# anguswilliams91/bpl-next

Hardware: NVIDIA B200
Metric: logdensity_grad_match_evals_per_s (higher is better)
Workload: dtype f32

## Files before the change

bpl_next_b200/csrc/api.cu:

```cuda
#include <limits.h>
#include <stdarg.h>
#include <stdlib.h>
#include <string.h>

#include <algorithm>
#include <atomic>
#include <mutex>
#include <new>

#include "common.cuh"
#include "plan.h"
#include "problem.h"
#include "loo.h"
#include "score_grid.h"
#include "simulate.h"

namespace bplx {

static thread_local char g_err[1024] = "";
static std::atomic<unsigned long long> g_launches{0};

void set_error(const char* fmt, ...) {
  va_list ap;
  va_start(ap, fmt);
// ... 216 lines not shown
  }
  p->kp = hp.kp;
  p->layout = hp.layout;
  p->lik_off = hp.lik_off;
  for (int i = 0; i < 12; i++) p->lik_hyper[i] = hp.lik_hyper[i];
  p->lik_nhyper = hp.lik_nhyper;
  p->lik_D = hp.lik_D;
  p->lik_const = hp.lik_const;
  p->lik_layout = hp.lik_layout;
  KernelParams& kp = p->kp;
#define UP(vec, ptr)                                 \
  if ((rc = upload(p, hp.vec, &(ptr))) != BPLX_OK) return fail(rc)
  UP(stream1, p->s1[0]);
  UP(stream2, p->s2[0]);
  UP(warp_b1, p->wb1[0]);
  UP(warp_b2, p->wb2[0]);
  for (int i = 1; i < kNumSplits; i++) {
    if (hp.more[i - 1].stream1.empty()) continue;
    UP(more[i - 1].stream1, p->s1[i]);
    UP(more[i - 1].stream2, p->s2[i]);
    UP(more[i - 1].warp_b1, p->wb1[i]);
    UP(more[i - 1].warp_b2, p->wb2[i]);
  }
  auto keep_bounds = [&](int i, const std::vector<uint32_t>& b1, const std::vector<uint32_t>& b2) {
    const size_t cap = sizeof(p->wb[i].b1) / sizeof(uint32_t);
    for (size_t k = 0; k < b1.size() && k < cap; k++) p->wb[i].b1[k] = b1[k];
    for (size_t k = 0; k < b2.size() && k < cap; k++) p->wb[i].b2[k] = b2[k];
  };
  keep_bounds(0, hp.warp_b1, hp.warp_b2);
  for (int i = 1; i < kNumSplits; i++) keep_bounds(i, hp.more[i - 1].warp_b1, hp.more[i - 1].warp_b2);
  kp.stream1 = p->s1[0];
  kp.stream2 = p->s2[0];
  kp.warp_b1 = p->wb1[0];
  kp.warp_b2 = p->wb2[0];
  kp.split = 1;
  UP(team_vptr, kp.team_vptr);
  UP(team_flags, kp.team_flags);
  UP(v_team, kp.v_team);
  UP(v_conf, kp.v_conf);
  UP(conf_vptr, kp.conf_vptr);
  UP(conf_vlist, kp.conf_vlist);
  UP(yexp, kp.yexp);
  UP(yteam, kp.yteam);
  UP(yconf, kp.yconf);
  UP(Xs, kp.Xs);
  UP(gw_tptr, kp.gw_tptr);
  UP(gw_tlist, kp.gw_tlist);
#undef UP
  rc = kp.model == BPLX_DYNAMIC ? logdensity_dynamic_set_attributes() : logdensity_set_attributes(kp);
  if (rc != BPLX_OK) return fail(rc);
  if (cudaDeviceGetAttribute(&p->sm_count, cudaDevAttrMultiProcessorCount, p->device) != cudaSuccess) p->sm_count = 0;
  p->max_clusters[0] = 1 << 30;
  if (kp.model != BPLX_DYNAMIC)
// ... 804 lines not shown
```

bpl_next_b200/csrc/k1_common.cuh:

```cuda
#pragma once
#include <float.h>

#include "common.cuh"
#include "plan.h"

namespace bplx {

namespace {


constexpr float kLn2 = 0.693147180559945309f;
constexpr unsigned kFull = 0xffffffffu;

struct Hyp {
  float mu_d, sig_a, sig_d, mu[4], sig[4];
};

struct Lane {
  const float* th;
  float* gr;
  float* sc;
  int sd;
  bool active;
  __device__ __forceinline__ float ld(int d) const { return __ldg(th + (uint32_t)(d * sd)); }
// ... 82 lines not shown
  const ThetaOffsets& o = kp.off;
  const float ra = g[eAh1] + g[eAa1] + g[eA0];
  const float rd = -(g[eBh1] + g[eBa1] + g[eB0]);
  const float rx[4] = {g[eAh1], g[eAa1], -g[eBh1], -g[eBa1]};
  if (kp.ndec == 0) hacc += rx[0];
  if (!ln.active) return;
  if (ADD) {
    red_add(ln.g(o.za + t), ra);
    red_add(ln.g(o.zd + t), rd);
  } else {
    *ln.g(o.za + t) = ra;
    *ln.g(o.zd + t) = rd;
  }
#pragma unroll
  for (int i = 0; i < 4; i++) {
    if (i < kp.ndec) {
      if (ADD) red_add(ln.g(o.dec[i] + t), rx[i]);
      else *ln.g(o.dec[i] + t) = rx[i];
    }
  }
}

__device__ __forceinline__ void put_side(const KernelParams& kp, float* q, const float (&g)[6], float& hacc) {
  q[0] = g[eAh1] + g[eAa1] + g[eA0];
  q[32] = -(g[eBh1] + g[eBa1] + g[eB0]);
  const float rx[4] = {g[eAh1], g[eAa1], -g[eBh1], -g[eBa1]};
  if (kp.ndec == 0) hacc += rx[0];
#pragma unroll
  for (int i = 0; i < 4; i++)
    if (i < kp.ndec) q[(2 + i) * 32] = rx[i];
}

struct Ring {
  uint32_t ring, bar;
  uint32_t S;
  const unsigned char* src;
  uint32_t total;
  uint32_t gs0, gs_next;
  int lane;

  __device__ __forceinline__ void init(uint32_t ring_, uint32_t bar_, uint32_t S_, int lane_) {
    ring = ring_; bar = bar_; S = S_; lane = lane_;
    total = gs0 = gs_next = 0;
    src = nullptr;
    if (lane == 0) {
#pragma unroll
      for (int s = 0; s < kStages; s++) mbar_init(bar + 8 * s, 1);
      fence_mbar_init();
      fence_proxy_async();
    }
    __syncwarp();
  }
  __device__ __forceinline__ void issue(uint32_t k) {
// ... 150 lines not shown
```

bpl_next_b200/csrc/logdensity.cu:

```cuda
#include <cooperative_groups.h>

#include <math.h>

#include "k1_common.cuh"
#include "problem.h"

namespace cg = cooperative_groups;

#ifdef BPLX_TIMELINE
__device__ unsigned long long g_timeline[32 * 24];
#define BPLX_STAMP(i)                                                                    \
  do {                                                                                   \
    if (blockIdx.x == 0 && (threadIdx.x & 31) == 0) {                                    \
      unsigned long long t_;                                                             \
      asm volatile("mov.u64 %0, %%globaltimer;" : "=l"(t_));                             \
      g_timeline[(threadIdx.x >> 5) * 24 + (i)] = t_;                                    \
    }                                                                                    \
  } while (0)
#define BPLX_STAMP_DEP(i, dep)                                                           \
  do {                                                                                   \
    if (blockIdx.x == 0 && (threadIdx.x & 31) == 0) {                                    \
      unsigned long long t_;                                                             \
      asm volatile("mov.u64 %0, %%globaltimer;" : "=l"(t_) : "f"(dep));                  \
      g_timeline[(threadIdx.x >> 5) * 24 + (i)] = t_;                                    \
    }                                                                                    \
// ... 60 lines not shown
    else __syncthreads();
  };
  const int chain_raw = group * kChains + lane;
  const int chain = min(chain_raw, kp.C - 1);
  Lane ln;
  ln.th = kp.theta + (size_t)chain * (size_t)kp.sc;
  ln.gr = kp.grad + (size_t)chain * (size_t)kp.sc;
  ln.sc = kp.scratch + chain;
  ln.sd = kp.sd;
  ln.active = chain_raw < kp.C;
  const uint32_t tab = smem_u32(smem) + lane * 8;
  unsigned long long* red_best = reinterpret_cast<unsigned long long*>(smem + kp.smem_red);
  unsigned long long* red_found = reinterpret_cast<unsigned long long*>(smem + kp.smem_red + 768);
  float* red_hyp = reinterpret_cast<float*>(smem + kp.smem_red + 1280);
  float* red_gc = reinterpret_cast<float*>(smem + kp.smem_red + 1280 + 12 * 128);
  const uint32_t a_best = cluster_map(smem_u32(red_best), 0), a_found = cluster_map(smem_u32(red_found), 0);
  const uint32_t a_cl = cluster_map(smem_u32(smem) + kp.smem_red_cl, 0);
  const uint32_t a_partcl = cluster_map(smem_u32(smem) + kp.epi_cl, 0);
  const uint32_t a_teamrows = cluster_map(smem_u32(smem) + kp.epi_team, 0);
  constexpr uint32_t ESZ = CLIP ? (uint32_t)sizeof(EntryClip) : (uint32_t)sizeof(Entry);
  Ring ring;
  ring.init(smem_u32(smem) + kp.smem_ring + warp * (kStages * kp.stage_bytes),
            smem_u32(smem) + kp.smem_bar + warp * (kStages * 8), kp.stage_bytes, lane);
  const uint32_t b1_0 = wb.b1[vwarp], b1_1 = wb.b1[vwarp + 1];
  ring.begin(kp.stream1 + b1_0, b1_1 - b1_0);
  pdl_wait();
  pdl_launch_dependents();
  ln.th = after_wait(ln.th);
  ln.gr = after_wait(ln.gr);
  ln.sc = after_wait(ln.sc);
  const int ndec = kp.ndec;
  const bool dc = ndec == 0;
  const float raw_in = ln.ld(o.raw);
  const bool lik = kp.lik_only != 0;
  const float u_in = (warp == 0 && !dc && !lik) ? ln.ld(o.u) : 0.0f;
  struct TeamIn { float za, zd, dz[4], xs[4]; int fl, v0, v1; };
  auto load_team = [&](int t) {
    TeamIn in;
    in.za = ln.ld(o.za + t);
    in.zd = ln.ld(o.zd + t);
#pragma unroll
    for (int i = 0; i < 4; i++) in.dz[i] = i < ndec ? ln.ld(o.dec[i] + t) : 0.0f;
#pragma unroll
    for (int j = 0; j < 4; j++) in.xs[j] = j < kp.K ? __ldg(kp.Xs + (size_t)t * kp.K + j) : 0.0f;
    in.fl = __ldg(kp.team_flags + t);
    in.v0 = __ldg(kp.team_vptr + t);
    in.v1 = __ldg(kp.team_vptr + t + 1);
    return in;
// ... 69 lines not shown
      for (int j = 0; j < 4; j++) {
        am = fmaf(in.xs[j], ba[j], am);
        dm = fmaf(in.xs[j], bd[j], dm);
      }
      for (int k = 4; k < kp.K; k++) {
        const float x = __ldg(kp.Xs + (size_t)t * kp.K + k);
        am = fmaf(x, ln.ld(o.beta_a + k), am);
        dm = fmaf(x, ln.ld(o.beta_d + k), dm);
      }
      const float att = fmaf(in.za, hy.sig_a, am), def = fmaf(in.zd, hy.sig_d, dm);
      float x[4] = {dc ? hy.mu[0] : 0.0f, 0.0f, 0.0f, 0.0f};
#pragma unroll
      for (int i = 0; i < 4; i++)
        if (i < ndec) x[i] = fmaf(hy.sig[i], in.dz[i], hy.mu[i]);
      if (!(in.fl & 1) && ln.active && crank == 0) {
        *ln.g(o.za + t) = 0.0f;
        *ln.g(o.zd + t) = 0.0f;
#pragma unroll
        for (int i = 0; i < 4; i++)
          if (i < ndec) *ln.g(o.dec[i] + t) = 0.0f;
      }
      for (int v = in.v0; v < in.v1; v++) {
        const float cf = kp.Cf > 0 ? ln.ld(o.conf + __ldg(kp.v_conf + v)) : 0.0f;
        float ex[6];
        ex[eAh1] = att + x[0] + cf;
        ex[eBh1] = -def - x[2] - cf;
        ex[eBa1] = -def - x[3] - cf;
        ex[eAa1] = att + x[1] + cf;
        ex[eA0] = att + cf;
        ex[eB0] = -def - cf;
        const uint32_t r = (uint32_t)v * kRowBytes;
        if (kp.has1) {
          sts64(tab + kp.tabP1 + r, expf(ex[eAh1]), expf(ex[eBh1]));
          sts64(tab + kp.tabQ1 + r, expf(ex[eBa1]), expf(ex[eAa1]));
        }
        if (kp.has0) sts64(tab + kp.tabP0 + r, expf(ex[eA0]), expf(ex[eB0]));
        if (CLIP) {
          exA = fmaxf(exA, fmaxf(ex[eAh1], fmaxf(ex[eAa1], ex[eA0])));
          exB = fmaxf(exB, fmaxf(ex[eBh1], fmaxf(ex[eBa1], ex[eB0])));
        }
        if (!CLIP && crank == 0) {
#pragma unroll
          for (int e = 0; e < 6; e++) lp_acc = fmaf(__ldg(kp.yexp + (size_t)v * 6 + e), ex[e], lp_acc);
        }
      }
    }
// ... 11 lines not shown
  bool fast1 = false;
  if (CLIP) fast1 = __all_sync(kFull, key_float(red_clip[lane]) + key_float(red_clip[32 + lane]) < 2.707f) && !(kp.force_clip_forms & 1);
  float best[3] = {0.0f, 0.0f, 0.0f};
  uint32_t besth[3] = {0u, 0u, 0u};
  {
    float g[6] = {0.0f, 0.0f, 0.0f, 0.0f, 0.0f, 0.0f}, cacc = 0.0f;
    const uint32_t nst = ring.num_stages();
    for (uint32_t k = 0; k < nst; k++) {
      uint32_t bytes;
      const uint32_t a0 = ring.acquire(k, &bytes);
      if (k == 0) BPLX_STAMP(16);
      uint32_t a = a0;
      const uint32_t aend = a0 + bytes;
      while (a + kp.min_piece1 <= aend) {
        const uint32_t hoff = b1_0 + k * ring.S + (a - a0);
        const Hdr L = unpack_hdr(lds128u(a));
        a += 16;
        const uint32_t e_end = a + L.n0 * ESZ;
        if (L.flags & kTeamFirst) {
#pragma unroll
          for (int e = 0; e < 6; e++) g[e] = 0.0f;
        }
        float2 own = lds64(tab + L.own_off);
        if (L.kind >= kH0) { const float s = own.x; own.x = own.y; own.y = s; }
        const bool home = (L.kind & 1) == 0;
        float gx, gy;
        if (!CLIP) {
          float2 acc0 = make_float2(0.0f, 0.0f), acc1 = acc0;
          if (home) {
            float m1 = 0.0f, m2 = 0.0f, m3 = 0.0f;
            walk16(a, e_end, [&](const uint32_t at) {
              const uint4 q = lds128u(at);
              const float2 ea = lds64(tab + q.x), eb = lds64(tab + q.z);
              acc0 = fma2(bc2(__uint_as_float(q.y)), ea, acc0);
              acc1 = fma2(bc2(__uint_as_float(q.w)), eb, acc1);
              m1 = fmaxf(m1, fmaxf(ea.x, eb.x));
              m2 = fmaxf(m2, fmaxf(ea.y, eb.y));
              m3 = fmaxf(m3, fmaxf(ea.x * ea.y, eb.x * eb.y));
            });
            const float v0 = own.x * m1, v1 = own.y * m2, v2 = (own.x * own.y) * m3;
            if (v0 > best[0]) { best[0] = v0; besth[0] = hoff; }
            if (v1 > best[1]) { best[1] = v1; besth[1] = hoff; }
            if (v2 > best[2]) { best[2] = v2; besth[2] = hoff; }
          } else {
            walk16(a, e_end, [&](const uint32_t at) {
              const uint4 q = lds128u(at);
              const float2 ea = lds64(tab + q.x), eb = lds64(tab + q.z);
              acc0 = fma2(bc2(__uint_as_float(q.y)), ea, acc0);
              acc1 = fma2(bc2(__uint_as_float(q.w)), eb, acc1);
            });
          }
          const float SX = own.x * (acc0.x + acc1.x), SY = own.y * (acc0.y + acc1.y);
          lp_acc -= 0.5f * (SX + SY);
          gx = -SX;
          gy = -SY;
        } else {
          float lp = 0.0f, m1 = 0.0f, m2 = 0.0f, m3 = 0.0f;
          if (fast1) {
            if (home) rate_piece_clip<true, true>(a, e_end, own, tab, lp, m1, m2, m3, gx, gy);
            else rate_piece_clip<true, false>(a, e_end, own, tab, lp, m1, m2, m3, gx, gy);
          } else {
            if (home) rate_piece_clip<false, true>(a, e_end, own, tab, lp, m1, m2, m3, gx, gy);
            else rate_piece_clip<false, false>(a, e_end, own, tab, lp, m1, m2, m3, gx, gy);
          }
          if (home) {
            lp_acc += lp;
            if (m1 > best[0]) { best[0] = m1; besth[0] = hoff; }
            if (m2 > best[1]) { best[1] = m2; besth[1] = hoff; }
            if (m3 > best[2]) { best[2] = m3; besth[2] = hoff; }
          }
        }
        add_own(g, L.kind, gx, gy);
        if (kp.Cf > 0) {
          cacc += L.kind == kH1 ? gx - gy : gy - gx;
          if (L.flags & kVteamLast) {
            if (ln.active) ln.sc[(size_t)L.vteam * kp.Cpad] = cacc;
            cacc = 0.0f;
          }
        }
        if (L.flags & kTeamLast) put_raw<false>(kp, ln, (int)L.team, g, hacc);
        if (k == 0 && a - a0 <= kp.stage_bytes / 2) BPLX_STAMP(17);
      }
      ring.release(k);
    }
  }
  const uint32_t b2_0 = wb.b2[vwarp], b2_1 = wb.b2[vwarp + 1];
  ring.begin(kp.stream2 + b2_0, b2_1 - b2_0);

  BPLX_STAMP(3);
#pragma unroll
  for (int q = 0; q < 3; q++)
    if (best[q] > 0.0f) dsm_atom_max_u32(a_best + (uint32_t)(q * 32 + lane) * 4u, __float_as_uint(best[q]));
  sync_all();
  BPLX_STAMP(14);
#pragma unroll
  for (int q = 0; q < 3; q++) {
    const float gq = __uint_as_float(dsm_ld_u32(a_best + (uint32_t)(q * 32 + lane) * 4u));
    if (best[q] == gq && gq > 0.0f) dsm_atom_min_u32(a_best + (uint32_t)((3 + q) * 32 + lane) * 4u, besth[q]);
    best[q] = gq;
  }
  sync_all();
  BPLX_STAMP(15);
#pragma unroll
  for (int q = 0; q < 3; q++) besth[q] = dsm_ld_u32(a_best + (uint32_t)((3 + q) * 32 + lane) * 4u);
  const bool noclip = CLIP && __all_sync(kFull, best[0] < 15.0f && best[1] < 15.0f) && !(kp.force_clip_forms & 2);
  const float Lam = fmaxf(best[0], best[1]);
  const int qlam = best[0] >= best[1] ? 0 : 1;
  bool s_need[2];
  uint32_t s_hoff[2], s_off0[2];
  uint4 s_hdr[2];
// ... 33 lines not shown
        float val;
        if (CLIP) {
          const float Xc = fminf(X, 15.0f), Yc = fminf(Y, 15.0f);
          val = q == 0 ? Xc : (q == 1 ? Yc : Xc * Yc);
        } else {
          val = q == 0 ? X : (q == 1 ? Y : (own.x * own.y) * (ea.x * ea.y));
        }
        if (val == target && found == 0xffffffffu) {
          found = (i << 24) | ((!CLIP || X < 15.0f) ? 1u << 23 : 0u) | ((!CLIP || Y < 15.0f) ? 1u << 22 : 0u) | off;
          info = L.vteam | (L.kind << 16);
        }
      }
    }
    if (found != 0xffffffffu) {
      dsm_atom_min_u32(a_found + (uint32_t)(which * 32 + lane) * 4u, found);
      dsm_st_u32(a_found + (uint32_t)(64 + which * 32 + lane) * 4u, info);
    }
  }

  BPLX_STAMP(5);
  float gc = 0.0f;
  {
    float g[6] = {0.0f, 0.0f, 0.0f, 0.0f, 0.0f, 0.0f}, cacc = 0.0f;
    const uint32_t nst = ring.num_stages();
    for (uint32_t k = 0; k < nst; k++) {
      uint32_t bytes;
      const uint32_t a0 = ring.acquire(k, &bytes);
      if (k == 0) BPLX_STAMP(18);
      uint32_t a = a0;
      const uint32_t aend = a0 + bytes;
      while (a + kp.min_piece2 <= aend) {
        const Hdr L = unpack_hdr(lds128u(a));
        a += 16;
        if (L.flags & kTeamFirst) {
#pragma unroll
          for (int e = 0; e < 6; e++) g[e] = 0.0f;
        }
        float2 own = lds64(tab + L.own_off);
        if (L.kind >= kH0) { const float s = own.x; own.x = own.y; own.y = s; }
        const bool home = (L.kind & 1) == 0;
        float lt, du, gx, gy;
        if (!CLIP) tau_piece<kTauPlain>(a, L, own, home, cc, tab, lt, du, gx, gy);
        else if (noclip) tau_piece<kTauUnclipped>(a, L, own, home, cc, tab, lt, du, gx, gy);
        else tau_piece<kTauClipped>(a, L, own, home, cc, tab, lt, du, gx, gy);
        if (home) {
          lp_acc = fmaf(lt, kLn2, lp_acc);
          gc += du;
        }
        add_own(g, L.kind, gx, gy);
        if (kp.Cf > 0) {
          cacc += L.kind == kH1 ? gx - gy : gy - gx;
          if (L.flags & kVteamLast) {
            if (ln.active) red_add(ln.sc + (size_t)L.vteam * kp.Cpad, cacc);
            cacc = 0.0f;
          }
        }
        if (L.flags & kTeamLast) {
          if (p2s) put_side(kp, p2_tab + (((L.kind & 1) * kp.T + L.team) * (2 + ndec)) * 32 + lane, g, hacc);
          else put_raw<true>(kp, ln, (int)L.team, g, hacc);
        }
      }
      ring.release(k);
    }
  }
  BPLX_STAMP(6);
  red_gc[warp * 32 + lane] = gc;
  __syncthreads();
  gc = 0.0f;
  for (int w = 0; w < W; w++) gc += red_gc[w * 32 + lane];
  if (S > 1) {
    if (warp == 0) dsm_st_f32(a_cl + (uint32_t)(crank * 32 + lane) * 4u, gc);
    cg::this_cluster().sync();
    gc = 0.0f;
    for (int q = 0; q < S; q++) gc += dsm_ld_f32(a_cl + (uint32_t)(q * 32 + lane) * 4u);
  }
  {
    const float t11 = fmaxf(1.0f - cc, 0.0f);
    gc -= kp.w11 / t11;
    if (vwarp == 0 && kp.w11 != 0.0f) lp_acc = fmaf(kp.w11, logf(t11), lp_acc);
  }

  BPLX_STAMP(7);
  Fixup fx;
  fx.h1 = 0u;
  fx.confs = 0u;
#pragma unroll
// ... 283 lines not shown
```

bpl_next_b200/csrc/plan.cc:

```cpp
#include "plan.h"

#include <algorithm>
#include <cmath>
#include <cstdarg>
#include <cstdio>
#include <cstdlib>
#include <cstring>
#include <map>
#include <numeric>

namespace bplx {
namespace {

struct RawEntry {
  uint32_t opp;
  uint8_t cls;
  double w, wyx, wyy;
};

std::string fmt(const char* f, ...) {
  char buf[512];
  va_list ap;
  va_start(ap, f);
  vsnprintf(buf, sizeof buf, f, ap);
// ... 309 lines not shown
  };
  auto opp_base = [&](int kind) -> uint32_t { return kind == kH1 ? kp.tabQ1 : kind == kA1 ? kp.tabP1 : kp.tabP0; };

  auto merge = [](std::vector<RawEntry>& v) {
    std::stable_sort(v.begin(), v.end(), [](const RawEntry& a, const RawEntry& b) {
      return a.cls != b.cls ? a.cls < b.cls : a.opp < b.opp;
    });
    size_t o = 0;
    for (size_t i = 0; i < v.size(); i++) {
      if (o && v[o - 1].cls == v[i].cls && v[o - 1].opp == v[i].opp) {
        v[o - 1].w += v[i].w;
        v[o - 1].wyx += v[i].wyx;
        v[o - 1].wyy += v[i].wyy;
      } else {
        v[o++] = v[i];
      }
    }
    v.resize(o);
  };
  for (auto& v : raw1) merge(v);
  for (auto& v : raw2) merge(v);
  P.team_flags.assign(T, 0);
  for (int v = 0; v < V; v++)
    for (int k = 0; k < 4; k++)
      if (!raw1[(size_t)v * 4 + k].empty()) P.team_flags[P.v_team[v]] |= 1;

  auto team_costs = [&](const std::vector<std::vector<RawEntry>>& raw, double per_entry, double per_list,
                        double per_team) {
    std::vector<double> cost(T, 0.0);
    for (int v = 0; v < V; v++)
      for (int k = 0; k < 4; k++) {
        const size_t n = raw[(size_t)v * 4 + k].size();
        if (n) cost[P.v_team[v]] += per_list * (1.0 + (double)n / 100.0) + per_entry * (double)n;
      }
    for (int t = 0; t < T; t++)
      if (cost[t] > 0.0) cost[t] += per_team;
    return cost;
  };
  auto assign = [&](const std::vector<double>& cost, int W, std::vector<std::vector<int>>* teams) {
    std::vector<int> order(T);
    std::iota(order.begin(), order.end(), 0);
    std::stable_sort(order.begin(), order.end(), [&](int a, int b) { return cost[a] > cost[b]; });
    std::vector<double> load(W, 0.0);
    teams->assign(W, {});
    for (int t : order) {
      if (cost[t] == 0.0) continue;
      int best = 0;
      for (int w = 1; w < W; w++)
        if (load[w] < load[best]) best = w;
      load[best] += cost[t];
      (*teams)[best].push_back(t);
    }
    for (auto& v : *teams) std::sort(v.begin(), v.end());
    return *std::max_element(load.begin(), load.end());
  };
  const std::vector<double> cost1 = team_costs(raw1, kp.clip ? 16.0 : 6.0, 40.0, 30.0);
  const std::vector<double> cost2 = team_costs(raw2, 12.0, 60.0, 30.0);
  auto smem_need = [&](int W, uint32_t stage) {
    const uint32_t epi = (K > 0 ? (uint32_t)T * kRowBytes : 0u) + (uint32_t)(W + kMaxSplit) * kPartRows * 128u;
    const uint32_t tabb = (std::max(table_bytes, epi) + 127u) / 128u * 128u;
    return tabb + (uint32_t)W * kStages * stage + 128u + (uint32_t)W * kStages * 8u + 3u * 256u + 2u * 128u + 2u * 128u +
           12u * 128u + (uint32_t)(W + kMaxSplit) * 128u;
  };
  const uint32_t kSmemMax = 227u * 1024u;
  int W = 0;
  uint32_t stage = 1024;
  std::vector<std::vector<int>> w1, w2;
  if (force_warps <= 0) {
    if (const char* e = getenv("BPLX_NWARPS")) force_warps = atoi(e);
  }
  if (const char* e = getenv("BPLX_STAGE")) stage = (uint32_t)atoi(e) == 512u ? 512u : 1024u;
  if (force_warps > 0) {
    W = std::max(1, std::min(force_warps, kMaxWarps));
    if (smem_need(W, stage) > kSmemMax) stage = 512;
  } else {
    double best = 0.0;
    for (int cand : {4, 8, 12, 16, 20, 24}) {
      if (cand > kMaxWarps) continue;
      uint32_t st = stage;
      if (smem_need(cand, st) > kSmemMax) st = 512;
// ... 3 lines not shown
      if (W == 0 || span < 0.97 * best) best = span, W = cand, stage = st;
    }
    if (W == 0) W = 4, stage = 512;
  }
  kp.nwarps = W;
  kp.stage_bytes = stage;
  kp.force_clip_forms = 0;
  if (const char* e = getenv("BPLX_CLIP_FORMS")) kp.force_clip_forms = atoi(e);
  {
    std::vector<std::vector<int>> t1, t2;
    const double span = assign(cost1, W, &t1) + assign(cost2, W, &t2);
    kp.split_hint = span >= 32000.0 ? 8 : span >= 16000.0 ? 4 : span >= 8000.0 ? 2 : 1;
  }

  std::vector<std::vector<int>> w2_items;
  kp.smem_p2 = 0;
  {
    std::vector<std::pair<int, double>> units;
    for (int t = 0; t < T; t++)
      for (int side = 0; side < 2; side++) {
        double c = 0.0;
        for (int v = P.team_vptr[t]; v < P.team_vptr[t + 1]; v++)
          for (int k = side; k < 4; k += 2) {
            const size_t n = raw2[(size_t)v * 4 + k].size();
            if (n) c += 60.0 * (1.0 + (double)n / 100.0) + 12.0 * (double)n;
          }
        if (c > 0.0) units.push_back({t * 4 + (1 << side), c + 30.0});
      }
    std::stable_sort(units.begin(), units.end(), [](const auto& a, const auto& b) { return a.second > b.second; });
    std::vector<double> load(W, 0.0);
    std::vector<std::vector<int>> items(W);
    for (const auto& u : units) {
      int best = 0;
      for (int w = 1; w < W; w++)
        if (load[w] < load[best]) best = w;
      load[best] += u.second;
      items[best].push_back(u.first);
    }
    for (auto& v : items) std::sort(v.begin(), v.end());
    std::vector<std::vector<int>> t2;
    const double span_team = assign(cost2, W, &t2);
    const double span_unit = units.empty() ? 0.0 : *std::max_element(load.begin(), load.end());
    const uint32_t p2_bytes = 2u * (uint32_t)T * (uint32_t)(2 + kp.ndec) * 128u;
    const bool off = getenv("BPLX_NO_P2SPLIT") != nullptr;
    if (!off && Cf <= 0 && span_unit < 0.85 * span_team && smem_need(W, stage) + p2_bytes <= kSmemMax) {
      w2_items = items;
      kp.smem_p2 = 1;
    }
  }

  const uint32_t zero_row = (uint32_t)V * kRowBytes;
  auto put = [](std::vector<unsigned char>* s, const void* p, size_t n) {
    const unsigned char* b = static_cast<const unsigned char*>(p);
    s->insert(s->end(), b, b + n);
  };
  auto emit = [&](int Wtot, std::vector<unsigned char>* s1, std::vector<unsigned char>* s2, std::vector<uint32_t>* wb1,
                  std::vector<uint32_t>* wb2) {
  const bool by_side = kp.smem_p2 != 0 && Wtot == kp.nwarps;
  const int W = Wtot;
  assign(cost1, W, &w1);
  assign(cost2, W, &w2);
  std::vector<std::vector<int>> it1(W), it2(W);
  for (int w = 0; w < W; w++) {
    for (int t : w1[w]) it1[w].push_back(t * 4 + 3);
    for (int t : w2[w]) it2[w].push_back(t * 4 + 3);
  }
  if (by_side) it2 = w2_items;
  P.n1 = P.n2 = P.n1_padded = P.n2_padded = P.nlists1 = P.nlists2 = 0;
  wb1->assign(W + 1, 0);
  wb2->assign(W + 1, 0);
  for (int phase = 1; phase <= 2; phase++) {
    const auto& raw = phase == 1 ? raw1 : raw2;
    const auto& by_warp = phase == 1 ? it1 : it2;
    std::vector<unsigned char>& S = phase == 1 ? *s1 : *s2;
    std::vector<uint32_t>& wb = phase == 1 ? *wb1 : *wb2;
    const size_t esz = (phase == 1 && kp.clip) ? sizeof(EntryClip) : sizeof(Entry);
    const size_t gran = 16;
    const size_t min_piece = sizeof(ListHdr) + gran;
    (phase == 1 ? kp.min_piece1 : kp.min_piece2) = (uint32_t)min_piece;
    S.clear();
    for (int w = 0; w < W; w++) {
      const size_t wstart = S.size();
      for (int item : by_warp[w]) {
        const int t = item >> 2, sides = item & 3;
        size_t team_first_hdr = (size_t)-1, last_hdr = 0;
        for (int v = P.team_vptr[t]; v < P.team_vptr[t + 1]; v++) {
          size_t vteam_last_hdr = (size_t)-1;
          for (int k = 0; k < 4; k++) {
            const auto& r = raw[(size_t)v * 4 + k];
            if (r.empty() || !((sides >> (k & 1)) & 1)) continue;
            (phase == 1 ? P.n1 : P.n2) += (long long)r.size();
            std::vector<unsigned char> body;
            std::vector<uint8_t> cls;
            if (phase == 1) {
              for (const RawEntry& e : r) {
                const uint32_t o = opp_base(k) + e.opp * kRowBytes;
                if (kp.clip) {
                  EntryClip x{o, (float)e.w, (float)e.wyx, (float)e.wyy};
                  put(&body, &x, sizeof x);
                } else {
                  Entry x{o, (float)e.w};
                  put(&body, &x, sizeof x);
                }
                cls.push_back(0);
              }
              while (!kp.clip && (cls.size() & 1)) {
                Entry x{opp_base(k) + zero_row, 0.0f};
                put(&body, &x, sizeof x);
                cls.push_back(0);
              }
            } else {
              size_t i = 0;
              for (int c = 0; c < 3; c++) {
                const uint32_t comp = c == 2 ? 4u : 0u;
                size_t cnt = 0;
                for (; i < r.size() && r[i].cls == c; i++, cnt++) {
                  Entry x{opp_base(k) + r[i].opp * kRowBytes + comp, (float)r[i].w};
                  put(&body, &x, sizeof x);
                  cls.push_back((uint8_t)c);
                }
                if (cnt & 1) {
                  Entry x{opp_base(k) + zero_row + comp, 0.0f};
                  put(&body, &x, sizeof x);
                  cls.push_back((uint8_t)c);
                }
              }
            }
            (phase == 1 ? P.n1_padded : P.n2_padded) += (long long)cls.size();
            size_t done = 0;
            while (done < cls.size()) {
              size_t in_stage = (S.size() - wstart) % stage;
              if (stage - in_stage < min_piece) {
                S.resize(S.size() + (stage - in_stage), 0);
                in_stage = 0;
              }
              const size_t space = stage - in_stage - sizeof(ListHdr);
              const size_t take = std::min(cls.size() - done, space / gran * gran / esz);
              ListHdr H{};
              H.own_off = own_off(v, k);
              H.vteam = (uint16_t)v;
              H.kind = (uint8_t)k;
              H.team = (uint16_t)t;
              uint16_t cnt[3] = {0, 0, 0};
              for (size_t i = done; i < done + take; i++) cnt[cls[i]]++;
              H.n0 = cnt[0];
              H.n1 = cnt[1];
              H.n2 = cnt[2];
              const size_t hdr_at = S.size();
              put(&S, &H, sizeof H);
              put(&S, body.data() + done * esz, take * esz);
              done += take;
              (phase == 1 ? P.nlists1 : P.nlists2)++;
              if (team_first_hdr == (size_t)-1) team_first_hdr = hdr_at;
              vteam_last_hdr = last_hdr = hdr_at;
            }
          }
          if (vteam_last_hdr != (size_t)-1) reinterpret_cast<ListHdr*>(&S[vteam_last_hdr])->flags |= kVteamLast;
        }
        if (team_first_hdr != (size_t)-1) {
          reinterpret_cast<ListHdr*>(&S[team_first_hdr])->flags |= kTeamFirst;
          reinterpret_cast<ListHdr*>(&S[last_hdr])->flags |= kTeamLast;
        }
      }
      wb[w + 1] = (uint32_t)S.size();
    }
    if (S.empty()) S.resize(16, 0);
  }
  };
  for (int i = kNumSplits - 1; i >= 1; i--)
    emit(W << i, &P.more[i - 1].stream1, &P.more[i - 1].stream2, &P.more[i - 1].warp_b1, &P.more[i - 1].warp_b2);
  emit(W, &P.stream1, &P.stream2, &P.warp_b1, &P.warp_b2);

  kp.epi_team = 0;
  kp.epi_part = K > 0 ? (uint32_t)T * kRowBytes : 0u;
  kp.epi_cl = kp.epi_part + (uint32_t)W * kPartRows * 128u;
  const uint32_t epi = kp.epi_cl + (uint32_t)kMaxSplit * kPartRows * 128u;
  kp.tab_bytes = (std::max(table_bytes, epi) + 127u) / 128u * 128u;
  kp.smem_ring = kp.tab_bytes;
  kp.smem_bar = kp.smem_ring + (uint32_t)W * kStages * stage;
  kp.smem_red = (kp.smem_bar + (uint32_t)W * kStages * 8u + 127u) / 128u * 128u;
  kp.smem_red_cl = kp.smem_red + 3u * 256u + 2u * 128u + 2u * 128u + 12u * 128u + (uint32_t)W * 128u;
  kp.smem_total = kp.smem_red_cl + (uint32_t)kMaxSplit * 128u;
  if (kp.smem_p2) {
    kp.smem_p2 = kp.smem_total;
    kp.smem_total += 2u * (uint32_t)T * (uint32_t)(2 + kp.ndec) * 128u;
  }
  if (kp.smem_total > kSmemMax)
    FAIL(BPLX_E_UNSUPPORTED, "problem needs %u bytes of shared memory per CTA (max %u): too many (team, confederation) pairs (%d)",
         kp.smem_total, kSmemMax, V);
#undef FAIL
  return BPLX_OK;
}

#include "plan_dynamic.inc"
// ... 3 lines not shown
```

bpl_next_b200/csrc/plan.h:

```cpp
#pragma once
#include <stdint.h>

#include <string>
#include <vector>

#include "../../include/bplx.h"

namespace bplx {

constexpr int kChains = 32;
constexpr int kRowBytes = 256;
constexpr int kMaxCov = 16;
constexpr int kMaxWarps = 24;
constexpr int kMaxWarpsDyn = 20;
constexpr int kStages = 2;
constexpr int kAccRows = 13;
constexpr int kPartRows = 16;
constexpr int kMaxSplit = 8;
constexpr int kNumSplits = 4;

enum Kind : uint8_t { kH1 = 0, kA1 = 1, kH0 = 2, kA0 = 3 };
enum Exponent : int { eAh1 = 0, eBh1 = 1, eBa1 = 2, eAa1 = 3, eA0 = 4, eB0 = 5 };

constexpr uint8_t kTeamFirst = 1;
constexpr uint8_t kTeamLast = 2;
constexpr uint8_t kVteamLast = 4;
constexpr uint8_t kGwFirst = 8;
constexpr uint8_t kStageEnd = 16;
constexpr uint8_t kPhase2 = 32;

struct Entry {
  uint32_t off;
  float w;
};
struct EntryClip {
  uint32_t off;
  float w;
  float wyx;
  float wyy;
};

struct ListHdr {
  uint32_t own_off;
  uint16_t vteam;
  uint8_t kind;
  uint8_t flags;
  uint16_t n0;
  uint16_t n1;
  uint16_t n2;
  uint16_t team;
};
static_assert(sizeof(ListHdr) == 16, "ListHdr must be 16 bytes");

struct ThetaOffsets {
  int mean_defence, log_std_attack, log_std_defence;
  int mean[4];
  int log_std[4];
  int u;
  int beta_a, beta_d;
  int za, zd;
  int dec[4];
  int conf;
  int raw;
};

struct HyperDesc {
  int off;
  int row;
  int kind;
  float loc, inv_scale;
};

struct WarpBounds {
  uint32_t b1[kMaxSplit * kMaxWarps + 1], b2[kMaxSplit * kMaxWarps + 1];
};

struct KernelParams {
  int model, T, K, Cf, V;
  int G;
  int as_written;
  int D, nwarps;
  int ndec;
  int clip;
  int lik_only;
  int has1, has0;
  uint32_t tabP1, tabQ1, tabP0;
  uint32_t tab_bytes;
  uint32_t stage_bytes;
  uint32_t min_piece1, min_piece2;
  uint32_t smem_ring, smem_bar, smem_red, smem_total;
  uint32_t epi_team, epi_part;
  uint32_t epi_cl;
  uint32_t smem_red_cl;
  uint32_t smem_p2;
  uint32_t dyn_state, dyn_part, dyn_hyp, dyn_fin;
  int dyn_nbuf;
  int dyn_hyp_ws;
// ... 14 lines not shown
  const float* yexp;
  const float* yteam;
  const float* yconf;
  const float* Xs;
  const int32_t* gw_tptr;
  const uint16_t* gw_tlist;
  HyperDesc hyper[12];
  int nhyper;
  float w11;
  float const_term;
  int C;
  int split;
  int sd, sc;
  const float* theta;
  float* lp;
  float* grad;
  float* corr_coef;
  float* scratch;
  int Cpad;
};

struct SplitStreams {
  std::vector<unsigned char> stream1, stream2;
  std::vector<uint32_t> warp_b1, warp_b2;
};

struct HostPlan {
  KernelParams kp{};
  ThetaOffsets lik_off{};
  HyperDesc lik_hyper[12]{};
  int lik_nhyper = 0, lik_D = 0;
  float lik_const = 0.0f;
  std::string lik_layout;
  std::vector<unsigned char> stream1, stream2;
  std::vector<uint32_t> warp_b1, warp_b2;
  SplitStreams more[kNumSplits - 1];
  std::vector<int32_t> team_vptr, conf_vptr, conf_vlist;
  std::vector<uint8_t> team_flags;
  std::vector<uint16_t> v_team;
  std::vector<uint8_t> v_conf;
  std::vector<float> yexp, yteam, yconf, Xs;
  std::vector<int32_t> gw_tptr;
  std::vector<uint16_t> gw_tlist;
  std::string layout;
  long long n1 = 0, n2 = 0, n1_padded = 0, n2_padded = 0, nlists1 = 0, nlists2 = 0;
};

int build_plan(const bplx_problem_desc& d, HostPlan* out, std::string* err, int force_warps = 0);

}
```

Before: 845.8 billion.

## Split rate phase into home and away sections, move away lists past reduction

The phase-1 stream is now split per warp into a home section and an away section, with a new per-warp boundary h1. Phase 1 before the global reduction walks only home lists, so the branch on home/away and the max tracking for away lists drop out of the critical pre-reduction loop. Away lists run after the reduction in the same pass as the tau lists, using new flag bits for team boundaries, and put_side now accumulates instead of overwriting. The planner's cost model is changed to balance work across the new phases. This adds stream padding and bookkeeping, and the change in accumulation semantics and scratch zeroing carries correctness risk.

```diff
diff --git a/bpl_next_b200/csrc/api.cu b/bpl_next_b200/csrc/api.cu
--- a/bpl_next_b200/csrc/api.cu
+++ b/bpl_next_b200/csrc/api.cu
@@ -262,13 +262,15 @@
     UP(more[i - 1].warp_b1, p->wb1[i]);
     UP(more[i - 1].warp_b2, p->wb2[i]);
   }
-  auto keep_bounds = [&](int i, const std::vector<uint32_t>& b1, const std::vector<uint32_t>& b2) {
+  auto keep_bounds = [&](int i, const std::vector<uint32_t>& b1, const std::vector<uint32_t>& b2,
+                         const std::vector<uint32_t>& h1) {
     const size_t cap = sizeof(p->wb[i].b1) / sizeof(uint32_t);
     for (size_t k = 0; k < b1.size() && k < cap; k++) p->wb[i].b1[k] = b1[k];
     for (size_t k = 0; k < b2.size() && k < cap; k++) p->wb[i].b2[k] = b2[k];
+    for (size_t k = 0; k < h1.size() && k + 1 < cap; k++) p->wb[i].h1[k] = h1[k];
   };
-  keep_bounds(0, hp.warp_b1, hp.warp_b2);
-  for (int i = 1; i < kNumSplits; i++) keep_bounds(i, hp.more[i - 1].warp_b1, hp.more[i - 1].warp_b2);
+  keep_bounds(0, hp.warp_b1, hp.warp_b2, hp.warp_h1);
+  for (int i = 1; i < kNumSplits; i++) keep_bounds(i, hp.more[i - 1].warp_b1, hp.more[i - 1].warp_b2, hp.more[i - 1].warp_h1);
   kp.stream1 = p->s1[0];
   kp.stream2 = p->s2[0];
   kp.warp_b1 = p->wb1[0];
diff --git a/bpl_next_b200/csrc/k1_common.cuh b/bpl_next_b200/csrc/k1_common.cuh
--- a/bpl_next_b200/csrc/k1_common.cuh
+++ b/bpl_next_b200/csrc/k1_common.cuh
@@ -128,13 +128,13 @@
 }
 
 __device__ __forceinline__ void put_side(const KernelParams& kp, float* q, const float (&g)[6], float& hacc) {
-  q[0] = g[eAh1] + g[eAa1] + g[eA0];
-  q[32] = -(g[eBh1] + g[eBa1] + g[eB0]);
+  q[0] += g[eAh1] + g[eAa1] + g[eA0];
+  q[32] += -(g[eBh1] + g[eBa1] + g[eB0]);
   const float rx[4] = {g[eAh1], g[eAa1], -g[eBh1], -g[eBa1]};
   if (kp.ndec == 0) hacc += rx[0];
 #pragma unroll
   for (int i = 0; i < 4; i++)
-    if (i < kp.ndec) q[(2 + i) * 32] = rx[i];
+    if (i < kp.ndec) q[(2 + i) * 32] += rx[i];
 }
 
 struct Ring {
diff --git a/bpl_next_b200/csrc/logdensity.cu b/bpl_next_b200/csrc/logdensity.cu
--- a/bpl_next_b200/csrc/logdensity.cu
+++ b/bpl_next_b200/csrc/logdensity.cu
@@ -1,6 +1,8 @@
 #include <cooperative_groups.h>
 
 #include <math.h>
+
+#include <type_traits>
 
 #include "k1_common.cuh"
 #include "problem.h"
@@ -107,8 +109,8 @@
   Ring ring;
   ring.init(smem_u32(smem) + kp.smem_ring + warp * (kStages * kp.stage_bytes),
             smem_u32(smem) + kp.smem_bar + warp * (kStages * 8), kp.stage_bytes, lane);
-  const uint32_t b1_0 = wb.b1[vwarp], b1_1 = wb.b1[vwarp + 1];
-  ring.begin(kp.stream1 + b1_0, b1_1 - b1_0);
+  const uint32_t b1_0 = wb.b1[vwarp], b1_1 = wb.b1[vwarp + 1], h1 = wb.h1[vwarp];
+  ring.begin(kp.stream1 + b1_0, h1 - b1_0);
   pdl_wait();
   pdl_launch_dependents();
   ln.th = after_wait(ln.th);
@@ -224,6 +226,7 @@
       }
       for (int v = in.v0; v < in.v1; v++) {
         const float cf = kp.Cf > 0 ? ln.ld(o.conf + __ldg(kp.v_conf + v)) : 0.0f;
+        if (kp.Cf > 0 && (in.fl & 2) && ln.active && crank == 0) ln.sc[(size_t)v * kp.Cpad] = 0.0f;
         float ex[6];
         ex[eAh1] = att + x[0] + cf;
         ex[eBh1] = -def - x[2] - cf;
@@ -281,53 +284,36 @@
           for (int e = 0; e < 6; e++) g[e] = 0.0f;
         }
         float2 own = lds64(tab + L.own_off);
-        if (L.kind >= kH0) { const float s = own.x; own.x = own.y; own.y = s; }
-        const bool home = (L.kind & 1) == 0;
+        if (L.kind == kH0) { const float s = own.x; own.x = own.y; own.y = s; }
         float gx, gy;
         if (!CLIP) {
           float2 acc0 = make_float2(0.0f, 0.0f), acc1 = acc0;
-          if (home) {
-            float m1 = 0.0f, m2 = 0.0f, m3 = 0.0f;
-            walk16(a, e_end, [&](const uint32_t at) {
-              const uint4 q = lds128u(at);
-              const float2 ea = lds64(tab + q.x), eb = lds64(tab + q.z);
-              acc0 = fma2(bc2(__uint_as_float(q.y)), ea, acc0);
-              acc1 = fma2(bc2(__uint_as_float(q.w)), eb, acc1);
-              m1 = fmaxf(m1, fmaxf(ea.x, eb.x));
-              m2 = fmaxf(m2, fmaxf(ea.y, eb.y));
-              m3 = fmaxf(m3, fmaxf(ea.x * ea.y, eb.x * eb.y));
-            });
-            const float v0 = own.x * m1, v1 = own.y * m2, v2 = (own.x * own.y) * m3;
-            if (v0 > best[0]) { best[0] = v0; besth[0] = hoff; }
-            if (v1 > best[1]) { best[1] = v1; besth[1] = hoff; }
-            if (v2 > best[2]) { best[2] = v2; besth[2] = hoff; }
-          } else {
-            walk16(a, e_end, [&](const uint32_t at) {
-              const uint4 q = lds128u(at);
-              const float2 ea = lds64(tab + q.x), eb = lds64(tab + q.z);
-              acc0 = fma2(bc2(__uint_as_float(q.y)), ea, acc0);
-              acc1 = fma2(bc2(__uint_as_float(q.w)), eb, acc1);
-            });
-          }
+          float m1 = 0.0f, m2 = 0.0f, m3 = 0.0f;
+          walk16(a, e_end, [&](const uint32_t at) {
+            const uint4 q = lds128u(at);
+            const float2 ea = lds64(tab + q.x), eb = lds64(tab + q.z);
+            acc0 = fma2(bc2(__uint_as_float(q.y)), ea, acc0);
+            acc1 = fma2(bc2(__uint_as_float(q.w)), eb, acc1);
+            m1 = fmaxf(m1, fmaxf(ea.x, eb.x));
+            m2 = fmaxf(m2, fmaxf(ea.y, eb.y));
+            m3 = fmaxf(m3, fmaxf(ea.x * ea.y, eb.x * eb.y));
+          });
+          const float v0 = own.x * m1, v1 = own.y * m2, v2 = (own.x * own.y) * m3;
+          if (v0 > best[0]) { best[0] = v0; besth[0] = hoff; }
+          if (v1 > best[1]) { best[1] = v1; besth[1] = hoff; }
+          if (v2 > best[2]) { best[2] = v2; besth[2] = hoff; }
           const float SX = own.x * (acc0.x + acc1.x), SY = own.y * (acc0.y + acc1.y);
           lp_acc -= 0.5f * (SX + SY);
           gx = -SX;
           gy = -SY;
         } else {
           float lp = 0.0f, m1 = 0.0f, m2 = 0.0f, m3 = 0.0f;
-          if (fast1) {
-            if (home) rate_piece_clip<true, true>(a, e_end, own, tab, lp, m1, m2, m3, gx, gy);
-            else rate_piece_clip<true, false>(a, e_end, own, tab, lp, m1, m2, m3, gx, gy);
-          } else {
-            if (home) rate_piece_clip<false, true>(a, e_end, own, tab, lp, m1, m2, m3, gx, gy);
-            else rate_piece_clip<false, false>(a, e_end, own, tab, lp, m1, m2, m3, gx, gy);
-          }
-          if (home) {
-            lp_acc += lp;
-            if (m1 > best[0]) { best[0] = m1; besth[0] = hoff; }
-            if (m2 > best[1]) { best[1] = m2; besth[1] = hoff; }
-            if (m3 > best[2]) { best[2] = m3; besth[2] = hoff; }
-          }
+          if (fast1) rate_piece_clip<true, true>(a, e_end, own, tab, lp, m1, m2, m3, gx, gy);
+          else rate_piece_clip<false, true>(a, e_end, own, tab, lp, m1, m2, m3, gx, gy);
+          lp_acc += lp;
+          if (m1 > best[0]) { best[0] = m1; besth[0] = hoff; }
+          if (m2 > best[1]) { best[1] = m2; besth[1] = hoff; }
+          if (m3 > best[2]) { best[2] = m3; besth[2] = hoff; }
         }
         add_own(g, L.kind, gx, gy);
         if (kp.Cf > 0) {
@@ -344,7 +330,8 @@
     }
   }
   const uint32_t b2_0 = wb.b2[vwarp], b2_1 = wb.b2[vwarp + 1];
-  ring.begin(kp.stream2 + b2_0, b2_1 - b2_0);
+  const uint32_t a1_0 = min(b1_0 + (h1 - b1_0 + ring.S - 1) / ring.S * ring.S, b1_1);
+  ring.begin(kp.stream1 + a1_0, b1_1 - a1_0);
 
   BPLX_STAMP(3);
 #pragma unroll
@@ -424,46 +411,75 @@
   float gc = 0.0f;
   {
     float g[6] = {0.0f, 0.0f, 0.0f, 0.0f, 0.0f, 0.0f}, cacc = 0.0f;
-    const uint32_t nst = ring.num_stages();
-    for (uint32_t k = 0; k < nst; k++) {
-      uint32_t bytes;
-      const uint32_t a0 = ring.acquire(k, &bytes);
-      if (k == 0) BPLX_STAMP(18);
-      uint32_t a = a0;
-      const uint32_t aend = a0 + bytes;
-      while (a + kp.min_piece2 <= aend) {
-        const Hdr L = unpack_hdr(lds128u(a));
-        a += 16;
-        if (L.flags & kTeamFirst) {
-#pragma unroll
-          for (int e = 0; e < 6; e++) g[e] = 0.0f;
-        }
-        float2 own = lds64(tab + L.own_off);
-        if (L.kind >= kH0) { const float s = own.x; own.x = own.y; own.y = s; }
-        const bool home = (L.kind & 1) == 0;
-        float lt, du, gx, gy;
-        if (!CLIP) tau_piece<kTauPlain>(a, L, own, home, cc, tab, lt, du, gx, gy);
-        else if (noclip) tau_piece<kTauUnclipped>(a, L, own, home, cc, tab, lt, du, gx, gy);
-        else tau_piece<kTauClipped>(a, L, own, home, cc, tab, lt, du, gx, gy);
-        if (home) {
-          lp_acc = fmaf(lt, kLn2, lp_acc);
-          gc += du;
-        }
-        add_own(g, L.kind, gx, gy);
-        if (kp.Cf > 0) {
-          cacc += L.kind == kH1 ? gx - gy : gy - gx;
-          if (L.flags & kVteamLast) {
-            if (ln.active) red_add(ln.sc + (size_t)L.vteam * kp.Cpad, cacc);
-            cacc = 0.0f;
+    auto walk = [&](auto tau_c) {
+      constexpr bool TAU = decltype(tau_c)::value;
+      const uint32_t nst = ring.num_stages();
+      for (uint32_t k = 0; k < nst; k++) {
+        uint32_t bytes;
+        const uint32_t a0 = ring.acquire(k, &bytes);
+        if (k == 0 && !TAU) BPLX_STAMP(18);
+        uint32_t a = a0;
+        const uint32_t aend = a0 + bytes;
+        while (a + kp.min_piece2 <= aend) {
+          const Hdr L = unpack_hdr(lds128u(a));
+          a += 16;
+          const uint32_t fl = TAU ? L.flags : L.flags >> 6;
+          if (fl & kTeamFirst) {
+#pragma unroll
+            for (int e = 0; e < 6; e++) g[e] = 0.0f;
           }
-        }
-        if (L.flags & kTeamLast) {
-          if (p2s) put_side(kp, p2_tab + (((L.kind & 1) * kp.T + L.team) * (2 + ndec)) * 32 + lane, g, hacc);
-          else put_raw<true>(kp, ln, (int)L.team, g, hacc);
-        }
-      }
-      ring.release(k);
-    }
+          float2 own = lds64(tab + L.own_off);
+          if (L.kind >= kH0) { const float s = own.x; own.x = own.y; own.y = s; }
+          float gx, gy;
+          if (TAU) {
+            const bool home = (L.kind & 1) == 0;
+            float lt, du;
+            if (!CLIP) tau_piece<kTauPlain>(a, L, own, home, cc, tab, lt, du, gx, gy);
+            else if (noclip) tau_piece<kTauUnclipped>(a, L, own, home, cc, tab, lt, du, gx, gy);
+            else tau_piece<kTauClipped>(a, L, own, home, cc, tab, lt, du, gx, gy);
+            if (home) {
+              lp_acc = fmaf(lt, kLn2, lp_acc);
+              gc += du;
+            }
+          } else {
+            const uint32_t e_end = a + L.n0 * ESZ;
+            if (!CLIP) {
+              float2 acc0 = make_float2(0.0f, 0.0f), acc1 = acc0;
+              walk16(a, e_end, [&](const uint32_t at) {
+                const uint4 q = lds128u(at);
+                const float2 ea = lds64(tab + q.x), eb = lds64(tab + q.z);
+                acc0 = fma2(bc2(__uint_as_float(q.y)), ea, acc0);
+                acc1 = fma2(bc2(__uint_as_float(q.w)), eb, acc1);
+              });
+              const float SX = own.x * (acc0.x + acc1.x), SY = own.y * (acc0.y + acc1.y);
+              lp_acc -= 0.5f * (SX + SY);
+              gx = -SX;
+              gy = -SY;
+            } else {
+              float lp, m1, m2, m3;
+              if (fast1) rate_piece_clip<true, false>(a, e_end, own, tab, lp, m1, m2, m3, gx, gy);
+              else rate_piece_clip<false, false>(a, e_end, own, tab, lp, m1, m2, m3, gx, gy);
+            }
+          }
+          add_own(g, L.kind, gx, gy);
+          if (kp.Cf > 0) {
+            cacc += L.kind == kH1 ? gx - gy : gy - gx;
+            if (L.flags & kVteamLast) {
+              if (ln.active) red_add(ln.sc + (size_t)L.vteam * kp.Cpad, cacc);
+              cacc = 0.0f;
+            }
+          }
+          if (fl & kTeamLast) {
+            if (p2s) put_side(kp, p2_tab + (((L.kind & 1) * kp.T + L.team) * (2 + ndec)) * 32 + lane, g, hacc);
+            else put_raw<true>(kp, ln, (int)L.team, g, hacc);
+          }
+        }
+        ring.release(k);
+      }
+    };
+    walk(std::false_type{});
+    ring.begin(kp.stream2 + b2_0, b2_1 - b2_0);
+    walk(std::true_type{});
   }
   BPLX_STAMP(6);
   red_gc[warp * 32 + lane] = gc;
diff --git a/bpl_next_b200/csrc/plan.cc b/bpl_next_b200/csrc/plan.cc
--- a/bpl_next_b200/csrc/plan.cc
+++ b/bpl_next_b200/csrc/plan.cc
@@ -355,19 +355,21 @@
   for (auto& v : raw2) merge(v);
   P.team_flags.assign(T, 0);
   for (int v = 0; v < V; v++)
-    for (int k = 0; k < 4; k++)
-      if (!raw1[(size_t)v * 4 + k].empty()) P.team_flags[P.v_team[v]] |= 1;
-
-  auto team_costs = [&](const std::vector<std::vector<RawEntry>>& raw, double per_entry, double per_list,
-                        double per_team) {
+    P.team_flags[P.v_team[v]] |= (raw1[(size_t)v * 4 + kH1].empty() && raw1[(size_t)v * 4 + kH0].empty()) ? 2 : 1;
+
+  const double kRateEntry = kp.clip ? 16.0 : 6.0, kRateList = 40.0, kTauEntry = 12.0, kTauList = 60.0, kTeamCost = 30.0;
+  auto list_cost = [&](size_t n, bool tau) {
+    return n == 0 ? 0.0 : (tau ? kTauList : kRateList) * (1.0 + (double)n / 100.0) + (tau ? kTauEntry : kRateEntry) * (double)n;
+  };
+  auto team_costs = [&](int phase) {
     std::vector<double> cost(T, 0.0);
     for (int v = 0; v < V; v++)
       for (int k = 0; k < 4; k++) {
-        const size_t n = raw[(size_t)v * 4 + k].size();
-        if (n) cost[P.v_team[v]] += per_list * (1.0 + (double)n / 100.0) + per_entry * (double)n;
+        if ((k & 1) == (phase == 1 ? 0 : 1)) cost[P.v_team[v]] += list_cost(raw1[(size_t)v * 4 + k].size(), false);
+        if (phase == 2) cost[P.v_team[v]] += list_cost(raw2[(size_t)v * 4 + k].size(), true);
       }
     for (int t = 0; t < T; t++)
-      if (cost[t] > 0.0) cost[t] += per_team;
+      if (cost[t] > 0.0) cost[t] += kTeamCost;
     return cost;
   };
   auto assign = [&](const std::vector<double>& cost, int W, std::vector<std::vector<int>>* teams) {
@@ -387,8 +389,7 @@
     for (auto& v : *teams) std::sort(v.begin(), v.end());
     return *std::max_element(load.begin(), load.end());
   };
-  const std::vector<double> cost1 = team_costs(raw1, kp.clip ? 16.0 : 6.0, 40.0, 30.0);
-  const std::vector<double> cost2 = team_costs(raw2, 12.0, 60.0, 30.0);
+  const std::vector<double> cost1 = team_costs(1), cost2 = team_costs(2);
   auto smem_need = [&](int W, uint32_t stage) {
     const uint32_t epi = (K > 0 ? (uint32_t)T * kRowBytes : 0u) + (uint32_t)(W + kMaxSplit) * kPartRows * 128u;
     const uint32_t tabb = (std::max(table_bytes, epi) + 127u) / 128u * 128u;
@@ -438,10 +439,10 @@
         double c = 0.0;
         for (int v = P.team_vptr[t]; v < P.team_vptr[t + 1]; v++)
           for (int k = side; k < 4; k += 2) {
-            const size_t n = raw2[(size_t)v * 4 + k].size();
-            if (n) c += 60.0 * (1.0 + (double)n / 100.0) + 12.0 * (double)n;
+            if (side == 1) c += list_cost(raw1[(size_t)v * 4 + k].size(), false);
+            c += list_cost(raw2[(size_t)v * 4 + k].size(), true);
           }
-        if (c > 0.0) units.push_back({t * 4 + (1 << side), c + 30.0});
+        if (c > 0.0) units.push_back({t * 4 + (1 << side), c + kTeamCost});
       }
     std::stable_sort(units.begin(), units.end(), [](const auto& a, const auto& b) { return a.second > b.second; });
     std::vector<double> load(W, 0.0);
@@ -470,8 +471,7 @@
     const unsigned char* b = static_cast<const unsigned char*>(p);
     s->insert(s->end(), b, b + n);
   };
-  auto emit = [&](int Wtot, std::vector<unsigned char>* s1, std::vector<unsigned char>* s2, std::vector<uint32_t>* wb1,
-                  std::vector<uint32_t>* wb2) {
+  auto emit = [&](int Wtot, SplitStreams* out) {
   const bool by_side = kp.smem_p2 != 0 && Wtot == kp.nwarps;
   const int W = Wtot;
   assign(cost1, W, &w1);
@@ -483,99 +483,118 @@
   }
   if (by_side) it2 = w2_items;
   P.n1 = P.n2 = P.n1_padded = P.n2_padded = P.nlists1 = P.nlists2 = 0;
-  wb1->assign(W + 1, 0);
-  wb2->assign(W + 1, 0);
+  out->warp_b1.assign(W + 1, 0);
+  out->warp_b2.assign(W + 1, 0);
+  out->warp_h1.assign(W, 0);
+  const size_t gran = 16;
+  const size_t min_piece = sizeof(ListHdr) + gran;
+  kp.min_piece1 = kp.min_piece2 = (uint32_t)min_piece;
+  ListHdr filler{};
+  filler.own_off = own_off(0, has1 ? kH1 : kH0);
+  filler.kind = (uint8_t)(has1 ? kH1 : kH0);
+  filler.team = P.v_team[0];
   for (int phase = 1; phase <= 2; phase++) {
-    const auto& raw = phase == 1 ? raw1 : raw2;
-    const auto& by_warp = phase == 1 ? it1 : it2;
-    std::vector<unsigned char>& S = phase == 1 ? *s1 : *s2;
-    std::vector<uint32_t>& wb = phase == 1 ? *wb1 : *wb2;
-    const size_t esz = (phase == 1 && kp.clip) ? sizeof(EntryClip) : sizeof(Entry);
-    const size_t gran = 16;
-    const size_t min_piece = sizeof(ListHdr) + gran;
-    (phase == 1 ? kp.min_piece1 : kp.min_piece2) = (uint32_t)min_piece;
+    std::vector<unsigned char>& S = phase == 1 ? out->stream1 : out->stream2;
+    std::vector<uint32_t>& wb = phase == 1 ? out->warp_b1 : out->warp_b2;
     S.clear();
     for (int w = 0; w < W; w++) {
       const size_t wstart = S.size();
-      for (int item : by_warp[w]) {
-        const int t = item >> 2, sides = item & 3;
-        size_t team_first_hdr = (size_t)-1, last_hdr = 0;
-        for (int v = P.team_vptr[t]; v < P.team_vptr[t + 1]; v++) {
-          size_t vteam_last_hdr = (size_t)-1;
-          for (int k = 0; k < 4; k++) {
-            const auto& r = raw[(size_t)v * 4 + k];
-            if (r.empty() || !((sides >> (k & 1)) & 1)) continue;
-            (phase == 1 ? P.n1 : P.n2) += (long long)r.size();
-            std::vector<unsigned char> body;
-            std::vector<uint8_t> cls;
-            if (phase == 1) {
-              for (const RawEntry& e : r) {
-                const uint32_t o = opp_base(k) + e.opp * kRowBytes;
-                if (kp.clip) {
-                  EntryClip x{o, (float)e.w, (float)e.wyx, (float)e.wyy};
+      for (int sec = 0; sec < (phase == 1 ? 2 : 1); sec++) {
+        const bool tau = phase == 2, away = sec == 1;
+        const uint8_t f_first = away ? kAwayFirst : kTeamFirst, f_last = away ? kAwayLast : kTeamLast;
+        const size_t sec_at = S.size();
+        if (away) {
+          const size_t in_stage = (S.size() - wstart) % stage;
+          if (in_stage && stage - in_stage < min_piece) S.resize(S.size() + (stage - in_stage), 0);
+          else if (in_stage) for (size_t b = in_stage; b < stage; b += sizeof filler) put(&S, &filler, sizeof filler);
+        }
+        const size_t body_at = S.size();
+        for (int item : (phase == 1 && !away) ? it1[w] : it2[w]) {
+          const int t = item >> 2, sides = item & 3;
+          size_t team_first_hdr = (size_t)-1, last_hdr = 0;
+          for (int v = P.team_vptr[t]; v < P.team_vptr[t + 1]; v++) {
+            size_t vteam_last_hdr = (size_t)-1;
+            for (int k = 0; k < 4; k++) {
+              if (!tau && (k & 1) != (away ? 1 : 0)) continue;
+              const auto& r = (tau ? raw2 : raw1)[(size_t)v * 4 + k];
+              if (r.empty() || !((sides >> (k & 1)) & 1)) continue;
+              (tau ? P.n2 : P.n1) += (long long)r.size();
+              const size_t esz = (!tau && kp.clip) ? sizeof(EntryClip) : sizeof(Entry);
+              std::vector<unsigned char> body;
+              std::vector<uint8_t> cls;
+              if (!tau) {
+                for (const RawEntry& e : r) {
+                  const uint32_t o = opp_base(k) + e.opp * kRowBytes;
+                  if (kp.clip) {
+                    EntryClip x{o, (float)e.w, (float)e.wyx, (float)e.wyy};
+                    put(&body, &x, sizeof x);
+                  } else {
+                    Entry x{o, (float)e.w};
+                    put(&body, &x, sizeof x);
+                  }
+                  cls.push_back(0);
+                }
+                while (!kp.clip && (cls.size() & 1)) {
+                  Entry x{opp_base(k) + zero_row, 0.0f};
                   put(&body, &x, sizeof x);
-                } else {
-                  Entry x{o, (float)e.w};
-                  put(&body, &x, sizeof x);
+                  cls.push_back(0);
                 }
-                cls.push_back(0);
-              }
-              while (!kp.clip && (cls.size() & 1)) {
-                Entry x{opp_base(k) + zero_row, 0.0f};
-                put(&body, &x, sizeof x);
-                cls.push_back(0);
-              }
-            } else {
-              size_t i = 0;
-              for (int c = 0; c < 3; c++) {
-                const uint32_t comp = c == 2 ? 4u : 0u;
-                size_t cnt = 0;
-                for (; i < r.size() && r[i].cls == c; i++, cnt++) {
-                  Entry x{opp_base(k) + r[i].opp * kRowBytes + comp, (float)r[i].w};
-                  put(&body, &x, sizeof x);
-                  cls.push_back((uint8_t)c);
-                }
-                if (cnt & 1) {
-                  Entry x{opp_base(k) + zero_row + comp, 0.0f};
-                  put(&body, &x, sizeof x);
-                  cls.push_back((uint8_t)c);
+              } else {
+                size_t i = 0;
+                for (int c = 0; c < 3; c++) {
+                  const uint32_t comp = c == 2 ? 4u : 0u;
+                  size_t cnt = 0;
+                  for (; i < r.size() && r[i].cls == c; i++, cnt++) {
+                    Entry x{opp_base(k) + r[i].opp * kRowBytes + comp, (float)r[i].w};
+                    put(&body, &x, sizeof x);
+                    cls.push_back((uint8_t)c);
+                  }
+                  if (cnt & 1) {
+                    Entry x{opp_base(k) + zero_row + comp, 0.0f};
+                    put(&body, &x, sizeof x);
+                    cls.push_back((uint8_t)c);
+                  }
                 }
               }
+              (tau ? P.n2_padded : P.n1_padded) += (long long)cls.size();
+              size_t done = 0;
+              while (done < cls.size()) {
+                size_t in_stage = (S.size() - wstart) % stage;
+                if (stage - in_stage < min_piece) {
+                  S.resize(S.size() + (stage - in_stage), 0);
+                  in_stage = 0;
+                }
+                const size_t space = stage - in_stage - sizeof(ListHdr);
+                const size_t take = std::min(cls.size() - done, space / gran * gran / esz);
+                ListHdr H{};
+                H.own_off = own_off(v, k);
+                H.vteam = (uint16_t)v;
+                H.kind = (uint8_t)k;
+                H.team = (uint16_t)t;
+                uint16_t cnt[3] = {0, 0, 0};
+                for (size_t i = done; i < done + take; i++) cnt[cls[i]]++;
+                H.n0 = cnt[0];
+                H.n1 = cnt[1];
+                H.n2 = cnt[2];
+                const size_t hdr_at = S.size();
+                put(&S, &H, sizeof H);
+                put(&S, body.data() + done * esz, take * esz);
+                done += take;
+                (phase == 1 ? P.nlists1 : P.nlists2)++;
+                if (team_first_hdr == (size_t)-1) team_first_hdr = hdr_at;
+                vteam_last_hdr = last_hdr = hdr_at;
+              }
             }
-            (phase == 1 ? P.n1_padded : P.n2_padded) += (long long)cls.size();
-            size_t done = 0;
-            while (done < cls.size()) {
-              size_t in_stage = (S.size() - wstart) % stage;
-              if (stage - in_stage < min_piece) {
-                S.resize(S.size() + (stage - in_stage), 0);
-                in_stage = 0;
-              }
-              const size_t space = stage - in_stage - sizeof(ListHdr);
-              const size_t take = std::min(cls.size() - done, space / gran * gran / esz);
-              ListHdr H{};
-              H.own_off = own_off(v, k);
-              H.vteam = (uint16_t)v;
-              H.kind = (uint8_t)k;
-              H.team = (uint16_t)t;
-              uint16_t cnt[3] = {0, 0, 0};
-              for (size_t i = done; i < done + take; i++) cnt[cls[i]]++;
-              H.n0 = cnt[0];
-              H.n1 = cnt[1];
-              H.n2 = cnt[2];
-              const size_t hdr_at = S.size();
-              put(&S, &H, sizeof H);
-              put(&S, body.data() + done * esz, take * esz);
-              done += take;
-              (phase == 1 ? P.nlists1 : P.nlists2)++;
-              if (team_first_hdr == (size_t)-1) team_first_hdr = hdr_at;
-              vteam_last_hdr = last_hdr = hdr_at;
-            }
+            if (vteam_last_hdr != (size_t)-1) reinterpret_cast<ListHdr*>(&S[vteam_last_hdr])->flags |= kVteamLast;
           }
-          if (vteam_last_hdr != (size_t)-1) reinterpret_cast<ListHdr*>(&S[vteam_last_hdr])->flags |= kVteamLast;
+          if (team_first_hdr != (size_t)-1) {
+            reinterpret_cast<ListHdr*>(&S[team_first_hdr])->flags |= f_first;
+            reinterpret_cast<ListHdr*>(&S[last_hdr])->flags |= f_last;
+          }
         }
-        if (team_first_hdr != (size_t)-1) {
-          reinterpret_cast<ListHdr*>(&S[team_first_hdr])->flags |= kTeamFirst;
-          reinterpret_cast<ListHdr*>(&S[last_hdr])->flags |= kTeamLast;
+        if (away) {
+          if (S.size() == body_at) S.resize(sec_at);
+          out->warp_h1[w] = (uint32_t)sec_at;
         }
       }
       wb[w + 1] = (uint32_t)S.size();
@@ -583,9 +602,16 @@
     if (S.empty()) S.resize(16, 0);
   }
   };
-  for (int i = kNumSplits - 1; i >= 1; i--)
-    emit(W << i, &P.more[i - 1].stream1, &P.more[i - 1].stream2, &P.more[i - 1].warp_b1, &P.more[i - 1].warp_b2);
-  emit(W, &P.stream1, &P.stream2, &P.warp_b1, &P.warp_b2);
+  for (int i = kNumSplits - 1; i >= 1; i--) emit(W << i, &P.more[i - 1]);
+  {
+    SplitStreams s1;
+    emit(W, &s1);
+    P.stream1 = std::move(s1.stream1);
+    P.stream2 = std::move(s1.stream2);
+    P.warp_b1 = std::move(s1.warp_b1);
+    P.warp_b2 = std::move(s1.warp_b2);
+    P.warp_h1 = std::move(s1.warp_h1);
+  }
 
   kp.epi_team = 0;
   kp.epi_part = K > 0 ? (uint32_t)T * kRowBytes : 0u;
diff --git a/bpl_next_b200/csrc/plan.h b/bpl_next_b200/csrc/plan.h
--- a/bpl_next_b200/csrc/plan.h
+++ b/bpl_next_b200/csrc/plan.h
@@ -28,6 +28,8 @@
 constexpr uint8_t kGwFirst = 8;
 constexpr uint8_t kStageEnd = 16;
 constexpr uint8_t kPhase2 = 32;
+constexpr uint8_t kAwayFirst = 64;
+constexpr uint8_t kAwayLast = 128;
 
 struct Entry {
   uint32_t off;
@@ -73,6 +75,7 @@
 
 struct WarpBounds {
   uint32_t b1[kMaxSplit * kMaxWarps + 1], b2[kMaxSplit * kMaxWarps + 1];
+  uint32_t h1[kMaxSplit * kMaxWarps];
 };
 
 struct KernelParams {
@@ -133,7 +136,7 @@
 
 struct SplitStreams {
   std::vector<unsigned char> stream1, stream2;
-  std::vector<uint32_t> warp_b1, warp_b2;
+  std::vector<uint32_t> warp_b1, warp_b2, warp_h1;
 };
 
 struct HostPlan {
@@ -144,7 +147,7 @@
   float lik_const = 0.0f;
   std::string lik_layout;
   std::vector<unsigned char> stream1, stream2;
-  std::vector<uint32_t> warp_b1, warp_b2;
+  std::vector<uint32_t> warp_b1, warp_b2, warp_h1;
   SplitStreams more[kNumSplits - 1];
   std::vector<int32_t> team_vptr, conf_vptr, conf_vlist;
   std::vector<uint8_t> team_flags;
```

Result: no change. 839.2 billion, median of 6 (-0.8%).
